# hal9000universe/deep-q-learning

Hardware: AMD Instinct MI355X
Metric: grad-updates/sec (higher is better)
Workload: dtype f32

## Files before the change

### deep-q-learning_amd/csrc/dqn_api.hip

```cpp
#include "../../include/dqn_hip.h"
#include "dqn_launch.h"
#include "dqn_per_device.h"

#include <dlfcn.h>
#include <cmath>
#include <cstdarg>
#include <cstdio>
#include <cstdlib>
#include <cstring>
#include <map>
#include <new>
#include <string>
#include <vector>

static thread_local std::string g_err;
thread_local hipEvent_t g_prof_ev0 = nullptr, g_prof_ev1 = nullptr;
static int fail(int code, const char *fmt, ...) {
    char buf[512];
    va_list ap; va_start(ap, fmt); vsnprintf(buf, sizeof(buf), fmt, ap); va_end(ap);
    g_err = buf;
    return code;
}
int dqn_set_error(int code, const char *msg) { g_err = msg; return code; }
#define HIP_TRY(expr)                                                                          \
// ... 22 lines not shown
struct Rccl {
    void *lib = nullptr;
    int (*GetUniqueId)(void *) = nullptr;
    int (*CommInitRank)(void **, int, NcclId, int) = nullptr;
    int (*AllReduce)(const void *, void *, size_t, int, int, void *, hipStream_t) = nullptr;
    int (*CommDestroy)(void *) = nullptr;
    int (*CommCount)(void *, int *) = nullptr;
    const char *(*GetErrorString)(int) = nullptr;
};

struct dqn_handle {
    dqn_config cfg;
    NetDims m;
    int L = 0;
    long long Ntree = 0;
    int Bp = 0;
    bool bf16 = false;
    void *arena = nullptr;
    size_t arena_bytes = 0, pack_bytes = 0;
    DqnState *st = nullptr;
    float *params = nullptr, *target = nullptr, *mu = nullptr, *nu = nullptr, *grad = nullptr;
    float *pack = nullptr, *pack_t = nullptr;
    float *pack_act = nullptr;
    float *states = nullptr, *observations = nullptr, *rewards = nullptr;
    int32_t *actions = nullptr; uint8_t *dones = nullptr;
    float *tree = nullptr; unsigned long long *stamp = nullptr;
    float *bs = nullptr, *bs2 = nullptr, *br = nullptr, *bw_raw = nullptr, *bisw = nullptr, *btd = nullptr,
          *btd_abs = nullptr, *bdf = nullptr;
    int32_t *ba = nullptr, *bidx = nullptr; uint8_t *bd = nullptr;
    float *q = nullptr, *nq = nullptr, *nt = nullptr;
    float *px = nullptr, *ph1 = nullptr, *ph2 = nullptr, *pdz1 = nullptr, *pdz2 = nullptr, *pdz3 = nullptr;
    float *loss_part = nullptr, *loss_dev = nullptr, *scratch = nullptr;
    int *tile_cnt = nullptr;
    float *big_slab = nullptr, *big_colsum = nullptr;
    float *pw_part = nullptr; int pw_force = 0;
    unsigned int *wmax_tmp = nullptr;
    int num_cus = 256;
    float *env_obs = nullptr, *env_next = nullptr, *env_r = nullptr; int32_t *env_a = nullptr; uint8_t *env_d = nullptr;
    float *hist_s = nullptr, *hist_r = nullptr; int32_t *hist_a = nullptr, *hist_d = nullptr;
    int n_step = 1; float gamma_n = 0.0f;
    bool no_handover = false;
    bool no_actor16 = false, f32_actor = false;
    bool big_any = false;
    int withhold = 0;
    int tile_stride = 0;
    float p_done = 0.01f;
    int env_kind = 0, env_max_steps = 500; int32_t *env_t = nullptr; float env_term_reward = 1.0f;
    bool env_time_feature = false;
    bool profiling = false;
    std::vector<hipEvent_t> events; size_t ev_used = 0;
    std::vector<const char *> ev_names;
    std::map<int, GraphSet> graphs;
    std::map<std::vector<int>, hipGraphExec_t> loop_graphs;
    void *comm = nullptr; int rank = 0, world = 1;
    std::map<int, std::pair<void *, int64_t>> bufs;
};

static Rccl g_rccl;

static size_t align_up(size_t x, size_t a) { return (x + a - 1) / a * a; }

static void L_pack(dqn_handle *h, hipStream_t s, const float *params, float *pack) {
    if (h->bf16) {
        launch_pack_bf16(s, h->m, params, pack);
        if (pack == h->pack) { launch_pack(s, h->m, params, h->pack_act); launch_pack_w2k16(s, h->m, params, h->pack_act); }
    } else launch_pack(s, h->m, params, pack);
}
static bool big_from(const dqn_handle *h, int B) { return h->big_any || (h->bf16 && B >= DQN_BIG_MIN_BF16); }
static bool use_big(dqn_handle *h, int B) { return h->big_slab != nullptr && big_supported(h->m, B, big_from(h, B)); }
static void L_fwd(dqn_handle *h, hipStream_t s, const FwdPass *p, int n, int B, const SampleArgs *smp = nullptr,
                  const BwdArgs *fuse = nullptr) {
    if (use_big(h, B) && !smp && !fuse) {
        bool plain = true;
        for (int i = 0; i < n; ++i) plain = plain && !p[i].act_out && !p[i].px && p[i].x;
        if (plain) { if (h->bf16) launch_big16_forward(s, h->m, p, n, B, h->num_cus); else launch_big_forward(s, h->m, p, n, B, h->num_cus); return; }
    }
    if (h->bf16) launch_qnet_fwd_bf16(s, h->m, p, n, B, smp, fuse, h->tile_cnt, h->st, h->tile_stride, h->withhold);
    else launch_qnet_fwd(s, h->m, p, n, B, smp, fuse, h->tile_cnt, h->st, h->tile_stride, h->withhold);
}
static void L_bwd(dqn_handle *h, hipStream_t s, const BwdArgs &g, int B) {
    if (h->bf16) launch_bwd_rows_bf16(s, h->m, g, B, h->st); else launch_bwd_rows(s, h->m, g, B, h->st);
}
static void L_dw(dqn_handle *h, hipStream_t s, int B, float *loss_out, int bump, const AdamArgs &ad, const PwArgs &pw) {
    if (h->bf16) launch_dw_bf16(s, h->m, h->px, h->ph1, h->ph2, h->pdz1, h->pdz2, h->pdz3, B, h->grad, h->loss_part, loss_out, h->st, bump, ad, pw);
    else launch_dw(s, h->m, h->px, h->ph1, h->ph2, h->pdz1, h->pdz2, h->pdz3, B, h->grad, h->loss_part, loss_out, h->st, bump, ad, pw);
}

static void arm(dqn_handle *h) {
    if (!h->profiling) return;
    while (h->events.size() < h->ev_used + 2) {
        hipEvent_t e;
        if (hipEventCreate(&e) != hipSuccess) return;
        h->events.push_back(e);
    }
    g_prof_ev0 = h->events[h->ev_used]; g_prof_ev1 = h->events[h->ev_used + 1];
}
static void mark(dqn_handle *h, hipStream_t st, const char *name) {
    (void)st;
    if (!h->profiling) return;
    h->ev_used += 2;
    h->ev_names.push_back(name);
}

extern "C" int dqn_create(const dqn_config *cfg, dqn_handle **out) {
    REQUIRE(cfg && out, "dqn_create: null argument");
    const int D = cfg->obs_dim, H1 = cfg->hidden1, H2 = cfg->hidden2, A = cfg->num_actions;
    REQUIRE(D >= 1 && D <= 256, "obs_dim %d out of range [1,256]", D);
    REQUIRE(H1 >= 16 && H1 <= 256 && H1 % 16 == 0, "hidden1 %d must be a multiple of 16 in [16,256]", H1);
    REQUIRE(H2 >= 16 && H2 <= 256 && H2 % 16 == 0, "hidden2 %d must be a multiple of 16 in [16,256]", H2);
    REQUIRE(A >= 1 && A <= 15, "num_actions %d out of range [1,15]", A);
    REQUIRE(cfg->capacity >= 1 && cfg->capacity <= (1ll << 30), "capacity out of range");
// ... 31 lines not shown
        if (L < 1) L = 1;
        h->L = L; h->Ntree = 1ll << L;
    }
    const long long N = cfg->capacity, P = h->m.P, Bp = h->Bp;
    const int K1 = h->m.KQ1 * 16;

    struct Item { void **p; size_t bytes; int id; };
    std::vector<Item> items;
    auto add = [&](void *pp, size_t bytes, int id = -1) { items.push_back({(void **)pp, bytes, id}); };
    add(&h->st, sizeof(DqnState));
    add(&h->params, P * 4, DQN_BUF_PARAMS); add(&h->target, P * 4, DQN_BUF_TARGET);
    add(&h->mu, P * 4, DQN_BUF_MU); add(&h->nu, P * 4, DQN_BUF_NU); add(&h->grad, P * 4, DQN_BUF_GRAD);
    const size_t esz = h->bf16 ? 2 : 4;
    const size_t pack_bytes = h->bf16 ? (size_t)bf16_pack_elems(h->m) * 2 : (size_t)h->m.pack_floats * 4;
    h->pack_bytes = pack_bytes;
    add(&h->pack, pack_bytes); add(&h->pack_t, pack_bytes);
    if (h->bf16) add(&h->pack_act, (size_t)h->m.pack_floats * 4 + (size_t)h->m.H1 * h->m.H2 * 2);
    add(&h->states, N * D * 4, DQN_BUF_STATES); add(&h->observations, N * D * 4, DQN_BUF_OBSERVATIONS);
    add(&h->rewards, N * 4, DQN_BUF_REWARDS); add(&h->actions, N * 4, DQN_BUF_ACTIONS);
    add(&h->dones, N, DQN_BUF_DONES);
    if (cfg->use_per) { add(&h->tree, 2 * h->Ntree * 4, DQN_BUF_TREE); add(&h->stamp, h->Ntree * 8); add(&h->pw_part, 8192 * 4); }
    add(&h->bs, Bp * D * 4); add(&h->bs2, Bp * D * 4); add(&h->br, Bp * 4); add(&h->bw_raw, Bp * 4);
    add(&h->bisw, Bp * 4, DQN_BUF_BATCH_ISW); add(&h->btd, Bp * 4, DQN_BUF_BATCH_TD); add(&h->btd_abs, Bp * 4);
    add(&h->bdf, Bp * 4); add(&h->ba, Bp * 4); add(&h->bidx, Bp * 4, DQN_BUF_BATCH_IDX); add(&h->bd, Bp);
    add(&h->q, Bp * A * 4); add(&h->nq, Bp * A * 4); add(&h->nt, Bp * A * 4);
    add(&h->px, Bp * (h->bf16 ? 32 : K1) * esz);
    add(&h->ph1, Bp * H1 * esz); add(&h->ph2, Bp * H2 * esz);
    add(&h->pdz1, Bp * H1 * esz); add(&h->pdz2, Bp * H2 * esz); add(&h->pdz3, Bp * 16 * esz);
    add(&h->loss_part, (Bp / 16) * 4); add(&h->loss_dev, 4, DQN_BUF_LOSS); add(&h->scratch, Bp * 4);
    if (big_supported(h->m, cfg->max_batch, big_from(h, cfg->max_batch))) {
        add(&h->big_slab, big_slab_floats(cfg->max_batch, h->num_cus) * 4); add(&h->big_colsum, big_colsum_floats(cfg->max_batch) * 4);
    }
    h->tile_stride = (int)(Bp / 16) + 2;
    add(&h->tile_cnt, (size_t)h->tile_stride * 2 * 4); add(&h->wmax_tmp, 4);
    add(&h->env_obs, Bp * D * 4, DQN_BUF_ENV_OBS); add(&h->env_next, Bp * D * 4); add(&h->env_r, Bp * 4);
    add(&h->env_a, Bp * 4, DQN_BUF_ENV_ACTIONS); add(&h->env_d, Bp); add(&h->env_t, Bp * 4);
    if (h->n_step > 1) {
        const size_t ns = (size_t)h->n_step;
        add(&h->hist_s, ns * Bp * D * 4); add(&h->hist_r, ns * Bp * 4); add(&h->hist_a, ns * Bp * 4); add(&h->hist_d, ns * Bp * 4);
    }
    size_t total = 0;
    for (auto &it : items) total += align_up(it.bytes, 256);
    hipError_t e = hipMalloc(&h->arena, total);
    if (e != hipSuccess) { delete h; return fail(DQN_ERR_NOMEM, "hipMalloc(%zu bytes): %s", total, hipGetErrorString(e)); }
    h->arena_bytes = total;
    e = hipMemset(h->arena, 0, total);
    if (e != hipSuccess) { (void)hipFree(h->arena); delete h; return fail(DQN_ERR_HIP, "hipMemset: %s", hipGetErrorString(e)); }
    size_t off = 0;
    for (auto &it : items) {
        *it.p = (char *)h->arena + off;
        if (it.id >= 0) h->bufs[it.id] = {*it.p, (int64_t)it.bytes};
        off += align_up(it.bytes, 256);
    }
    DqnState s0{};
    s0.b1pow = 1.0; s0.b2pow = 1.0; s0.pmax = 1.0f; s0.beta = cfg->per_beta; s0.lr = cfg->lr;
    e = hipMemcpy(h->st, &s0, sizeof(s0), hipMemcpyHostToDevice);
    if (e != hipSuccess) { (void)hipFree(h->arena); delete h; return fail(DQN_ERR_HIP, "state init: %s", hipGetErrorString(e)); }
    *out = h;
    return DQN_OK;
}

static void destroy_graphs(dqn_handle *h) {
    for (auto &kv : h->graphs) {
        if (kv.second.fused) (void)hipGraphExecDestroy(kv.second.fused);
        if (kv.second.bwd) (void)hipGraphExecDestroy(kv.second.bwd);
        if (kv.second.apply) (void)hipGraphExecDestroy(kv.second.apply);
        if (kv.second.actor) (void)hipGraphExecDestroy(kv.second.actor);
// ... 341 lines not shown
            mark(h, st, "big_fwd2");
            g.nq = h->nq; g.nt = h->nt;
            arm(h);
            launch_big16_rows_bwd(st, h->m, p + 2, 1, B, g, h->px, h->ph1, h->ph2, h->big_colsum, h->st, h->num_cus);
        } else launch_big_rows_bwd(st, h->m, p, 3, B, g, h->px, h->ph1, h->ph2, h->big_colsum, h->st, h->num_cus);
        mark(h, st, "big_rows_fwd3_bwd");
        arm(h);
        (h->bf16 ? launch_big16_dw : launch_big_dw)(st, h->m, h->px, h->ph1, h->ph2, h->pdz1, h->pdz2, h->pdz3, B, h->big_slab, h->big_colsum, h->grad,
                      h->loss_part, h->loss_dev, h->st, 1, fuse_adam ? adam_args(h) : AdamArgs{}, h->num_cus);
        mark(h, st, "big_dw");
        if (fuse_pw && h->cfg.use_per) enqueue_per_writeback(h, B, st);
        (void)defer_top;
        return;
    }
    SampleArgs sm{};
    sm.st = h->st; sm.tree = h->cfg.use_per ? h->tree : nullptr; sm.N = h->Ntree; sm.L = h->L;
    sm.states = h->states; sm.observations = h->observations; sm.rewards = h->rewards; sm.actions = h->actions;
    sm.dones = h->dones; sm.seed = h->cfg.seed;
    sm.idx = h->bidx; sm.a = h->ba; sm.r = h->br; sm.w_raw = h->bw_raw; sm.d = h->bd;
    sm.pre = presampled ? 1 : 0;
    FwdPass p[3] = { make_pass(h, DQN_NET_ONLINE, nullptr, h->q, nullptr, true),
                     make_pass(h, DQN_NET_ONLINE, nullptr, h->nq, nullptr, false),
                     make_pass(h, DQN_NET_TARGET, nullptr, h->nt, nullptr, false) };
    p[0].src = 1; p[1].src = 2; p[2].src = 2;
    BwdArgs g{};
    g.q = h->q; g.nq = h->nq; g.nt = h->nt; g.a = h->ba; g.r = h->br; g.d_u8 = h->bd;
    g.w_raw = h->cfg.use_per ? h->bw_raw : nullptr;
    g.gamma = h->n_step > 1 ? h->gamma_n : h->cfg.gamma;
    g.ph1 = h->ph1; g.ph2 = h->ph2; g.pack = h->pack;
    g.pdz1 = h->pdz1; g.pdz2 = h->pdz2; g.pdz3 = h->pdz3;
    g.td = h->btd; g.td_abs = h->btd_abs; g.isw_out = h->bisw; g.loss_part = h->loss_part;
    const int grid_tiles = h->bf16 ? 2 * ((B + 31) / 32) : (B + 15) / 16;
    const bool fuse_rows = 3 * grid_tiles <= h->num_cus && (presampled || !h->cfg.use_per) && !h->no_handover;
    if (fuse_rows) p[0].q = nullptr;
    arm(h);
    L_fwd(h, st, p, 3, B, &sm, fuse_rows ? &g : nullptr);
    mark(h, st, fuse_rows ? "sample_fwd_x3_bwd" : "sample_fwd_x3");
    if (!fuse_rows) {
        arm(h);
        L_bwd(h, st, g, B);
        mark(h, st, "td_bwd_rows");
    }
    PwArgs pw{};
    if (fuse_pw && h->cfg.use_per)
        pw = PwArgs{h->tree, h->Ntree, h->L, h->bidx, h->btd_abs, B, h->cfg.per_alpha, h->cfg.per_eps};
    arm(h);
    L_dw(h, st, B, h->loss_dev, 1, fuse_adam ? adam_args(h) : AdamArgs{}, pw);
    mark(h, st, fuse_adam ? (pw.tree ? "dw_adam_perwrite" : "dw_adam") : (pw.tree ? "dw_perwrite" : "dw"));
    if (pw.tree && !defer_top) { arm(h); launch_per_top(st, h->st, h->tree, h->L); mark(h, st, "per_top"); }
}

static void enqueue_apply(dqn_handle *h, int B, hipStream_t st) {
    (void)B;
    arm(h);
    enqueue_adam(h, st);
    mark(h, st, "adam");
}

static void enqueue_update(dqn_handle *h, int B, hipStream_t st, bool capturing, bool defer_top = false,
                           bool presampled = false) {
    (void)capturing;
    if (h->world == 1) {
        enqueue_backward(h, B, st, true, true, defer_top, presampled);
    } else {
        enqueue_backward(h, B, st, false, true, false, presampled);
        enqueue_apply(h, B, st);
    }
// ... 310 lines not shown

extern "C" int dqn_allreduce_grads(dqn_handle *h, void *stream) {
    REQUIRE(h, "null argument");
    if (!h->comm) return fail(DQN_ERR_STATE, "dqn_allreduce_grads before dqn_comm_init");
    const int e = g_rccl.AllReduce(h->grad, h->grad, (size_t)h->m.P,  7,  0, h->comm,
                                   (hipStream_t)stream);
    if (e) return fail(DQN_ERR_COMM, "ncclAllReduce: %s", g_rccl.GetErrorString ? g_rccl.GetErrorString(e) : "?");
    return DQN_OK;
}

extern "C" int dqn_comm_count_host(dqn_handle *h, int32_t *ranks) {
    REQUIRE(h && ranks, "null argument");
    *ranks = 0;
    if (!h->comm) return DQN_OK;
    if (!g_rccl.CommCount) return fail(DQN_ERR_COMM, "librccl.so lacks ncclCommCount");
    int n = 0;
    const int e = g_rccl.CommCount(h->comm, &n);
    if (e) return fail(DQN_ERR_COMM, "ncclCommCount: %s", g_rccl.GetErrorString ? g_rccl.GetErrorString(e) : "?");
    *ranks = n;
    return DQN_OK;
}

extern "C" int dqn_debug_withhold_handover(dqn_handle *h, int32_t on) {
    REQUIRE(h, "null handle");
    HIP_TRY(hipDeviceSynchronize());
    destroy_graphs(h);
    h->withhold = on ? 1 : 0;
    return DQN_OK;
}

extern "C" int dqn_clear_device_errors(dqn_handle *h) {
    REQUIRE(h, "null handle");
    HIP_TRY(hipDeviceSynchronize());
    if (h->tile_cnt) HIP_TRY(hipMemset(h->tile_cnt, 0, (size_t)h->tile_stride * 2 * 4));
    const unsigned int z = 0;
    HIP_TRY(hipMemcpy(&h->st->err_count, &z, 4, hipMemcpyHostToDevice));
    HIP_TRY(hipMemcpy(&h->st->arrive, &z, 4, hipMemcpyHostToDevice));
    HIP_TRY(hipMemcpy(&h->st->fill_cnt, &z, 4, hipMemcpyHostToDevice));
    return DQN_OK;
}

extern "C" int dqn_device_errors_host(dqn_handle *h, int64_t *count) {
    REQUIRE(h && count, "null argument");
    unsigned int c = 0;
    HIP_TRY(hipDeviceSynchronize());
    HIP_TRY(hipMemcpy(&c, &h->st->err_count, 4, hipMemcpyDeviceToHost));
    *count = (int64_t)c;
    return DQN_OK;
}
```

### deep-q-learning_amd/csrc/dqn_device.h

```cpp
#pragma once
#include <hip/hip_runtime.h>
#include <stdint.h>

#define LDS_BARRIER() asm volatile("s_waitcnt lgkmcnt(0)\n\ts_barrier" ::: "memory")

struct DqnState {
    unsigned long long ring_counter;
    long long          size;
    unsigned long long sample_ctr;
    unsigned long long epoch;
    unsigned long long env_ctr;
    double             b1pow, b2pow;
    int                adam_count;
    float              pmax;
    float              beta;
    float              lr;
    float              loss;
    float              wmax;
    float              epsilon;
    float              pad0;
    unsigned int       arrive;
    unsigned int       pad;
    unsigned long long ep_count;
    unsigned long long ep_steps;
// ... 58 lines not shown
    p = p * z; p = p + 1.0f;
    const float ln_m = (2.0f * s) * p;
    const float r = ln_m * 1.44269502f;
    return (float)e + r;
}

__device__ __forceinline__ float exp2_det(float y) {
    const float fi = floorf(y + 0.5f);
    int i = (int)fi;
    const float f = y - fi;
    const float t = f * 0.693147182f;
    float p = 1.98412701e-4f;
    p = p * t; p = p + 1.38888892e-3f;
    p = p * t; p = p + 8.33333377e-3f;
    p = p * t; p = p + 4.16666679e-2f;
    p = p * t; p = p + 0.166666672f;
    p = p * t; p = p + 0.5f;
    p = p * t; p = p + 1.0f;
    p = p * t; p = p + 1.0f;
    i = i < -126 ? -126 : (i > 127 ? 127 : i);
    return p * __uint_as_float((uint32_t)(i + 127) << 23);
}

__device__ __forceinline__ float pow_det(float x, float a) { return exp2_det(a * log2_det(x)); }

__device__ __forceinline__ unsigned int ticket_take_early(unsigned int *p, unsigned int v) {
    __attribute__((address_space(1))) unsigned int *g = (__attribute__((address_space(1))) unsigned int *)p;
    asm volatile("" : "+v"(g));
    return __hip_atomic_fetch_add(g, v, __ATOMIC_RELAXED, __HIP_MEMORY_SCOPE_AGENT);
}

#ifdef DQN_STAMPS
extern __device__ unsigned long long g_stamps[8][64][2];
#define STAMP(K, S)                                                                         \
    do { if (threadIdx.x == 0 && blockIdx.x == 0 && blockIdx.y == 0) {                       \
             g_stamps[K][S][0] = __builtin_amdgcn_s_memtime();                                \
             g_stamps[K][S][1] = __builtin_amdgcn_s_memrealtime(); } } while (0)
#else
#define STAMP(K, S) do { } while (0)

#endif
```

### deep-q-learning_amd/csrc/dqn_launch.h

```cpp
#pragma once
#include <hip/hip_runtime.h>
#include <stdint.h>
#include "dqn_device.h"

#include <hip/hip_ext.h>

int dqn_set_error(int code, const char *msg);

struct EnvArgs;
struct SampleArgs;

extern thread_local hipEvent_t g_prof_ev0, g_prof_ev1;
#define DQN_LAUNCH(kernel, grid, block, lds, stream, ...)                                                    \
    do {                                                                                                      \
        if (g_prof_ev0) {                                                                                     \
            hipExtLaunchKernelGGL(kernel, grid, block, lds, stream, g_prof_ev0, g_prof_ev1, 0, __VA_ARGS__); \
            g_prof_ev0 = nullptr; g_prof_ev1 = nullptr;                                                       \
        } else {                                                                                              \
            hipLaunchKernelGGL(kernel, grid, block, lds, stream, __VA_ARGS__);                                \
        }                                                                                                     \
    } while (0)

struct NetDims {
    int D, H1, H2, A;
// ... 1 lines not shown
    long long o_w1, o_b1, o_w2, o_b2, o_wv, o_bv, o_wa, o_ba, P;
    long long p_w1, p_w2, p_wh, p_w2t, p_wht, pack_floats;
    long long p_w2k;
};
NetDims make_dims(int D, int H1, int H2, int A);

struct FwdPass {
    const float *x;
    const float *params;
    const float *pack;
    float *q;
    float *feat;
    float *px, *ph1, *ph2;
    int src;
    int32_t *act_out;
    const DqnState *act_state;
    float act_eps; unsigned long long act_seed, act_ctr;
};

struct BwdArgs {
    const float *q, *nq, *nt;
    const float *targets;
    const int32_t *a; const float *r; const uint8_t *d_u8; const float *d_f32;
    const float *w_raw;
    const float *isw;
    float gamma;
    const float *ph1, *ph2;
    const float *pack;
    float *pdz1, *pdz2, *pdz3;
    float *td, *td_abs, *dq, *targets_out, *isw_out;
    float *loss_part;
};

struct FuseBwd { BwdArgs g; int *tile_cnt; DqnState *st; int tiles; int withhold; };

struct PwArgs {
    float *tree; long long N; int L; const int32_t *idx; const float *td_abs; int B; float alpha, eps;
};
struct AdamArgs {
    float *P, *mu, *nu, *pack; int adamw; float b1, b2, eps, wd, grad_scale;
    float *pack_act;
};

void launch_pack(hipStream_t s, const NetDims &m, const float *params, float *pack);
void launch_pack_w2k16(hipStream_t s, const NetDims &m, const float *params, float *pack_act);
void launch_qnet_fwd(hipStream_t s, const NetDims &m, const FwdPass *passes, int npass, int B, const SampleArgs *smp = nullptr,
                     const BwdArgs *fuse = nullptr, int *tile_cnt = nullptr, DqnState *st = nullptr, int tile_stride = 0, int withhold = 0);
bool actor_multi_supported(const NetDims &m, int n_envs, int T);
bool launch_actor_multi(hipStream_t s, const NetDims &m, const EnvArgs &env, int T, const float *params, const float *pack,
                        int32_t *act_out, int B, const SampleArgs *smp, bool bf16, int num_cus, bool no_wide);
void launch_td(hipStream_t s, const float *q, const float *nq, const float *nt, const int32_t *a,
               const float *r, const float *d, const float *isw, float gamma, int B, int A,
               float *targets, float *td, float *dq, float *loss, float *scratch);
void launch_loss(hipStream_t s, const float *pred, const float *targets, const float *isw, int B, int A,
                 float *loss);
void launch_bwd_rows(hipStream_t s, const NetDims &m, const BwdArgs &g, int B, DqnState *st);
void launch_dw(hipStream_t s, const NetDims &m, const float *px, const float *ph1, const float *ph2,
               const float *pdz1, const float *pdz2, const float *pdz3, int B, float *grad,
               const float *loss_part, float *loss_out, DqnState *st, int bump_ctr, const AdamArgs &adam,
               const PwArgs &pw = PwArgs{});
void launch_per_top(hipStream_t st_, DqnState *st, float *tree, int L);
void launch_adam(hipStream_t s, const NetDims &m, DqnState *st, float *params, const float *grad, float *mu,
                 float *nu, float *pack, int adamw, float b1, float b2, float eps, float wd, float grad_scale);
void launch_policy(hipStream_t s, const float *q, int n, int A, float epsilon, unsigned long long seed,
                   unsigned long long ctr, int32_t *actions, const DqnState *st_from);
void launch_u8_to_f32(hipStream_t s, const uint8_t *in, float *out, int n);

#define DQN_BIG_MIN 16384
#define DQN_BIG_MIN_BF16 8192
#define DQN_BIG_MAX_SLICES 64
bool big_supported(const NetDims &m, int B, bool any_size = false);
size_t big_slab_floats(int max_batch, int num_cus);
size_t big_colsum_floats(int max_batch);
int big_dw_slices(int B, int num_cus);
int dqn_rccl_comm_init(void **comm, const void *unique_id_128, int rank, int world);
int dqn_rccl_allreduce_sum_f32(void *comm, float *buf, size_t n, hipStream_t st);
void dqn_rccl_comm_destroy(void *comm);
int dqn_rccl_comm_count(void *comm, int *n);
void launch_big_forward(hipStream_t s, const NetDims &m, const FwdPass *passes, int npass, int B, int num_cus);
void launch_big16_forward(hipStream_t s, const NetDims &m, const FwdPass *passes, int npass, int B, int num_cus);
// ... 47 lines not shown
```

### deep-q-learning_amd/csrc/dqn_net.hip

```cpp
#include <type_traits>
#include "dqn_device.h"
#include "dqn_launch.h"
#include "dqn_per_device.h"
#include "dqn_net_common.h"


#ifdef DQN_STAMPS
__device__ unsigned long long g_stamps[8][64][2];
extern "C" int dqn_debug_stamps(unsigned long long *out_host) {
    return (int)hipMemcpyFromSymbol(out_host, HIP_SYMBOL(g_stamps), sizeof(g_stamps));
}
#endif

#define MFMA4(a, b, c) __builtin_amdgcn_mfma_f32_16x16x4f32((a), (b), (c), 0, 0, 0)

__device__ __forceinline__ int perm16(int c) { return ((c & 3) << 2) | (c >> 2); }


__device__ __forceinline__ int pfrag(int KQb, int tile, int ct, int r, int lane) {
    return (ct * KQb + tile) * 256 + r * 64 + ((lane & 15) << 2) + (lane >> 4);
}

NetDims make_dims(int D, int H1, int H2, int A) {
    NetDims m{};
// ... 57 lines not shown
struct MmaLayer {
    static constexpr int AHEAD = PF >= 16 ? 6 : PF;
    const float4 *pk[TN];
    float4 b0[PF][TN], b1[PP ? PF : 1][PP ? TN : 1];
    int KQ, CT, wave;

    template <int R, int C>
    __device__ __forceinline__ void load(float4 (&b)[R][C], int kq0) {
#pragma unroll
        for (int p = 0; p < PF; ++p) {
            int kq = kq0 + p;
            kq = kq < KQ ? kq : KQ - 1;
#pragma unroll
            for (int t = 0; t < TN; ++t) b[p][t] = pk[t][(long long)kq * 64];
        }
    }
    template <int R, int C>
    __device__ __forceinline__ void compute(const float4 (&b)[R][C], int kq0, const float *arow, f32x4 (&acc)[TN]) {
#pragma unroll
        for (int p = 0; p < PF; ++p) {
            const int kq = kq0 + p;
            if (kq < KQ) {
                const float4 a4 = *reinterpret_cast<const float4 *>(arow + 16 * kq);
#pragma unroll
                for (int t = 0; t < TN; ++t) {
                    acc[t] = MFMA4(a4.x, b[p][t].x, acc[t]);
                    acc[t] = MFMA4(a4.y, b[p][t].y, acc[t]);
                    acc[t] = MFMA4(a4.z, b[p][t].z, acc[t]);
                    acc[t] = MFMA4(a4.w, b[p][t].w, acc[t]);
                }
            }
        }
    }
    __device__ __forceinline__ void init(const float *__restrict__ pack, int KQ_, int CT_, int wave_, int lane) {
        KQ = KQ_; CT = CT_; wave = wave_;
#pragma unroll
        for (int t = 0; t < TN; ++t) {
            int ct = wave + 4 * t;
            ct = ct < CT ? ct : CT - 1;
            pk[t] = reinterpret_cast<const float4 *>(pack) + (long long)ct * KQ * 64 + lane;
        }
    }
    template <int P0, int P1>
    __device__ __forceinline__ void load_range() {
#pragma unroll
        for (int p = P0; p < P1; ++p) {
            int kq = p < KQ ? p : KQ - 1;
#pragma unroll
            for (int t = 0; t < TN; ++t) b0[p][t] = pk[t][(long long)kq * 64];
        }
    }
    __device__ __forceinline__ void start(const float *__restrict__ pack, int KQ_, int CT_, int wave_, int lane) {
        init(pack, KQ_, CT_, wave_, lane);
        load(b0, 0);
    }
    __device__ __forceinline__ void finish_heads4(const float *lds_a, int stride, int lane, f32x4 &out) {
        static_assert(TN == 1 && !PP, "heads: one tile, single chunk");
        f32x4 c0 = {0.f, 0.f, 0.f, 0.f}, c1 = c0, c2 = c0, c3 = c0;
        const float *arow = lds_a + (lane & 15) * stride + 4 * (lane >> 4);
        float4 a_cur = *reinterpret_cast<const float4 *>(arow);
#pragma unroll
        for (int p = 0; p < PF; ++p) {
            if (p < KQ) {
                const float4 a4 = a_cur;
                if (p + 1 < PF) a_cur = *reinterpret_cast<const float4 *>(arow + (p + 1 < KQ ? 16 * (p + 1) : 0));
                c0 = MFMA4(a4.x, b0[p][0].x, c0);
                c1 = MFMA4(a4.y, b0[p][0].y, c1);
                c2 = MFMA4(a4.z, b0[p][0].z, c2);
                c3 = MFMA4(a4.w, b0[p][0].w, c3);
                __builtin_amdgcn_sched_barrier(0);
            }
// ... 41 lines not shown
struct FwdPasses { FwdPass p[3]; };


template <int TN1, int TN2, bool FUSE>
__global__ void __launch_bounds__(256)
k_qnet_fwd(NetDims m, FwdPasses passes, int B, SampleArgs smp, FuseBwd fb) {
    extern __shared__ __attribute__((aligned(16))) float lds[];
    const FwdPass ps = passes.p[blockIdx.y];
    const int tile = blockIdx.x, row0 = tile * 16;
    const int tid = threadIdx.x, wave = tid >> 6, lane = tid & 63;
    const int KQb = (B + 15) / 16;
    const int K1 = m.KQ1 * 16;
    const int sx = K1 + 4, s1 = m.H1 + 4, s2 = m.H2 + 4;
    float *lx = lds, *l1 = lx + 16 * sx, *l2 = l1 + 16 * s1, *lh = l2 + 16 * s2;

    STAMP(0, 0);
    const bool sampling = smp.st != nullptr;
    int *lidx = reinterpret_cast<int *>(lh + 256 + 16);
    const float *ring = sampling ? (ps.src == 1 ? smp.states : smp.observations) : nullptr;
    auto xload = [&](int t) -> float {
        const int rl = t / K1, c = t - rl * K1;
        if (!(t < 16 * K1 && row0 + rl < B && c < m.D)) return 0.0f;
        return sampling ? ring[(long long)lidx[rl] * m.D + c] : ps.x[(long long)(row0 + rl) * m.D + c];
    };
    float xv[4];
    if (!sampling) {
#pragma unroll
        for (int u = 0; u < 4; ++u) xv[u] = xload(tid + 256 * u);
    }
    const bool presampled = sampling && smp.pre;
    int pre_leaf = 0;
    if (presampled && tid < 16) pre_leaf = smp.idx[row0 + tid < B ? row0 + tid : B - 1];
    MmaLayer<TN1, 2, true> L1; MmaLayer<TN2, 16, false> L2; MmaLayer<1, 16, false> LH;
    MmaLayer<TN2, 1, false> LA; MmaLayer<TN1, 16, false> LB;
    L1.start(ps.pack + m.p_w1, m.KQ1, m.H1 / 16, wave, lane);
    float bias1[TN1], bias2[TN2], biash = 0.0f;
#pragma unroll
    for (int t = 0; t < TN1; ++t) { int ct = wave + 4 * t; ct = ct < m.H1 / 16 ? ct : m.H1 / 16 - 1; bias1[t] = ps.params[m.o_b1 + 16 * ct + (lane & 15)]; }
#pragma unroll
    for (int t = 0; t < TN2; ++t) { int ct = wave + 4 * t; ct = ct < m.H2 / 16 ? ct : m.H2 / 16 - 1; bias2[t] = ps.params[m.o_b2 + 16 * ct + (lane & 15)]; }
    if (wave == 0) {
        const int c = lane & 15;
        if (c == 0) biash = ps.params[m.o_bv];
        else if (c <= m.A) biash = ps.params[m.o_ba + c - 1];
    }
    int row_a = 0; float row_r = 0.0f; int row_d = 0;
    if (presampled) {
        if (tid < 16) {
            lidx[tid] = pre_leaf;
            const int k = row0 + tid;
            if (blockIdx.y == 0 && k < B) {
                row_a = smp.actions[pre_leaf]; row_r = smp.rewards[pre_leaf]; row_d = smp.dones[pre_leaf];
                smp.a[k] = row_a; smp.r[k] = row_r; smp.d[k] = (uint8_t)row_d;
            }
        }
        LDS_BARRIER();
#pragma unroll
        for (int u = 0; u < 4; ++u) xv[u] = xload(tid + 256 * u);
    }
    L2.init(ps.pack + m.p_w2, m.H1 / 16, m.H2 / 16, wave, lane);
    L2.template load_range<0, 6>();
    if (wave == 0) LH.init(ps.pack + m.p_wh, m.H2 / 16, 1, 0, lane);
    if (sampling && !presampled) {
        if (smp.tree) {
            float *lsub = reinterpret_cast<float *>(lidx + 16);
            sample_tile_coop(smp, row0, B, tid, blockIdx.y == 0, lidx, lsub, lsub + 512);
        } else {
            if (tid < 16) sample_tile(smp, row0, B, tid, blockIdx.y == 0, lidx);
            LDS_BARRIER();
        }
#pragma unroll
        for (int u = 0; u < 4; ++u) xv[u] = xload(tid + 256 * u);
        if constexpr (FUSE) {
            if (blockIdx.y == 0 && tid < 16 && row0 + tid < B) {
                const int leaf = lidx[tid];
                row_a = smp.actions[leaf]; row_r = smp.rewards[leaf]; row_d = smp.dones[leaf];
            }
        }
    }

#pragma unroll
    for (int u = 0; u < 4; ++u) {
        const int t = tid + 256 * u;
        if (t < 16 * K1) {
            const int rl = t / K1, c = t - rl * K1;
            lx[rl * sx + (c & ~15) + perm16(c & 15)] = xv[u];
        }
    }
    for (int t = tid + 1024; t < 16 * K1; t += 256) {
        const int rl = t / K1, c = t - rl * K1;
        const float v = xload(t);
        lx[rl * sx + (c & ~15) + perm16(c & 15)] = v;
    }
    LDS_BARRIER();
    STAMP(0, 1);

    unsigned m1bits = 0u, m2bits = 0u;
    {
        f32x4 acc[TN1];
        L1.finish(lx, sx, lane, acc);
        STAMP(0, 11);
#pragma unroll
        for (int t = 0; t < TN1; ++t) {
            const int ct = wave + 4 * t;
            if (ct < m.H1 / 16) {
                const int c = lane & 15;
                const float bias = bias1[t];
// ... 6 lines not shown
                    l1[rl * s1 + 16 * ct + perm16(c)] = v;
                }
            }
        }
    }
    STAMP(0, 12);
    if (wave == 0) LH.template load_range<0, 16>();
    STAMP(0, 13);
    LDS_BARRIER();
    STAMP(0, 2);

    {
        f32x4 acc[TN2];
        L2.finish(l1, s1, lane, acc);
        STAMP(0, 3);
#pragma unroll
        for (int t = 0; t < TN2; ++t) {
            const int ct = wave + 4 * t;
            if (ct < m.H2 / 16) {
                const int c = lane & 15, col = 16 * ct + c;
                const float bias = bias2[t];
#pragma unroll
                for (int r = 0; r < 4; ++r) {
                    const int rl = 4 * (lane >> 4) + r;
                    float v = acc[t][r] + bias;
                    v = v > 0.0f ? v : 0.0f;
                    if constexpr (FUSE) m2bits |= (v > 0.0f ? 1u : 0u) << (4 * t + r);
                    l2[rl * s2 + 16 * ct + perm16(c)] = v;
                    if (ps.feat && row0 + rl < B) ps.feat[(long long)(row0 + rl) * m.H2 + col] = v;
                }
            }
        }
    }
    LDS_BARRIER();
    STAMP(0, 4);

    if (ps.px && wave != 0) {
        auto stash = [&](float *dst, const float *img, int stride, int CT) {
            float4 *out = reinterpret_cast<float4 *>(dst);
            for (int q = tid - 64; q < CT * 64; q += 192) {
                const int ct = q >> 6, lp = q & 63;
                const float *col = img + (lp >> 4) * stride + 16 * ct + perm16(lp & 15);
                out[(long long)(ct * KQb + tile) * 64 + lp] = float4{col[0], col[4 * stride], col[8 * stride], col[12 * stride]};
            }
        };
        stash(ps.px, lx, sx, m.KQ1);
        stash(ps.ph1, l1, s1, m.H1 / 16);
        stash(ps.ph2, l2, s2, m.H2 / 16);
    }
    if (wave == 0) {
        f32x4 acc;
        LH.finish_heads4(l2, s2, lane, acc);
        const int c = lane & 15;
#pragma unroll
        for (int r = 0; r < 4; ++r) lh[(4 * (lane >> 4) + r) * 16 + c] = acc[r] + biash;
    }
    if constexpr (FUSE) {
        if (blockIdx.y == 0) {
            LA.start(fb.g.pack + m.p_wht, 1, m.H2 / 16, wave, lane);
            LB.init(fb.g.pack + m.p_w2t, m.H2 / 16, m.H1 / 16, wave, lane);
            LB.template load_range<0, 16>();
        }
    }
    LDS_BARRIER();
    STAMP(0, 5);

    float qrow[16];
    if (tid < 16 && row0 + tid < B) {
        const float *hr = lh + tid * 16;
        float sum = 0.0f;
        if constexpr (FUSE) {
            if (m.A <= 4) {
#pragma unroll
                for (int a = 0; a < 4; ++a) if (a < m.A) sum = sum + hr[1 + a];
            } else {
#pragma unroll
                for (int a = 0; a < 15; ++a) if (a < m.A) sum = sum + hr[1 + a];
            }
        } else {
            for (int a = 0; a < m.A; ++a) sum = sum + hr[1 + a];
        }
        const float mean = __fdiv_rn(sum, (float)m.A);
        if constexpr (FUSE) {
#pragma unroll
            for (int a = 0; a < 15; ++a) qrow[a] = a < m.A ? (hr[0] + hr[1 + a]) - mean : 0.0f;
        } else {
            for (int a = 0; a < m.A; ++a) qrow[a] = (hr[0] + hr[1 + a]) - mean;
        }
        if constexpr (FUSE) {
            if (blockIdx.y != 0) {
#pragma unroll
                for (int a = 0; a < 15; ++a) asm volatile("" : "+v"(qrow[a]));
#pragma unroll
                for (int a = 0; a < 15; ++a)
                    if (a < m.A) __hip_atomic_store(&ps.q[(long long)(row0 + tid) * m.A + a], qrow[a], __ATOMIC_RELAXED, __HIP_MEMORY_SCOPE_AGENT);
            } else if (ps.q) {
#pragma unroll
                for (int a = 0; a < 15; ++a) if (a < m.A) ps.q[(long long)(row0 + tid) * m.A + a] = qrow[a];
            }
        } else if (ps.q) for (int a = 0; a < m.A; ++a) ps.q[(long long)(row0 + tid) * m.A + a] = qrow[a];
        if (ps.act_out) {
            const float eps = ps.act_state ? ps.act_state->epsilon : ps.act_eps;
            const unsigned long long ctr = ps.act_state ? ps.act_state->env_ctr : ps.act_ctr;
            const int act = policy_row(qrow, m.A, eps, ps.act_seed, ctr, row0 + tid);
            ps.act_out[row0 + tid] = act;
        }
    }
    STAMP(0, 6);
    if constexpr (FUSE) {
        if (blockIdx.y != 0) {
            if (wave == 0) {
                asm volatile("s_waitcnt vmcnt(0)" ::: "memory");
                if (tid == 0) atomicAdd(reinterpret_cast<unsigned *>(fb.tile_cnt) + tile, fb.withhold ? 0u : 1u);
            }
            return;
        }
        const BwdArgs &g = fb.g;
        const int A = m.A;
        const int s3 = 16 + 4;
        float *l3 = lx;
        float *lz2 = lh + 256 + 32 + 528, *lrow = lz2 + 16 * s2;
        const int irow = row0 + tid;
        const bool rowt = tid < 16 && irow < B;
        float wi = 1.0f, wmax = 1.0f;
        if (rowt && g.w_raw) { wi = g.w_raw[irow]; wmax = fb.st->wmax; }
        for (int t = tid; t < 16 * s3; t += 256) l3[t] = 0.0f;
        bool gave_up = false;
        if (tid == 0) {
            unsigned *cnt = reinterpret_cast<unsigned *>(fb.tile_cnt) + tile, *seen = reinterpret_cast<unsigned *>(fb.tile_cnt) + fb.tiles + tile;
            const unsigned want = *seen + 2u;
            if (!wait_word_eq(cnt, want, 2)) { flag_wait_timeout(fb.st); gave_up = true; }
            *seen = want;
        }
        LDS_BARRIER();
        STAMP(0, 7);
        if (tid < 16) {
            float rowloss = 0.0f;
            if (rowt) {
                auto td_rows = [&](auto amax_tag) {
                constexpr int AMAX = decltype(amax_tag)::value;
                float nqr[AMAX], ntr[AMAX];
#pragma unroll
                for (int k2 = 0; k2 < AMAX; ++k2) {
                    nqr[k2] = k2 < A ? __hip_atomic_load(&g.nq[(long long)irow * A + k2], __ATOMIC_RELAXED, __HIP_MEMORY_SCOPE_AGENT) : 0.0f;
                    ntr[k2] = k2 < A ? __hip_atomic_load(&g.nt[(long long)irow * A + k2], __ATOMIC_RELAXED, __HIP_MEMORY_SCOPE_AGENT) : 0.0f;
                }
                float w = 1.0f;
                if (g.w_raw) w = __fdiv_rn(wi, wmax);
                const float invB = __fdiv_rn(1.0f, (float)B);
                float best = nqr[0], nt_star = ntr[0], q_a = qrow[0];
#pragma unroll
                for (int k2 = 1; k2 < AMAX; ++k2) {
                    if (k2 < A && nqr[k2] > best) { best = nqr[k2]; nt_star = ntr[k2]; }
                    if (k2 == row_a) q_a = qrow[k2];
                }
                const float di = row_d ? 1.0f : 0.0f;
                const float t1 = g.gamma * nt_star;
                const float t2 = t1 - q_a;
                const float t3 = (1.0f - di) * t2;
                float delta = row_r + t3, dabs = fabsf(delta);
                asm volatile("" : "+v"(delta), "+v"(dabs), "+v"(w));
                if (g.w_raw && g.isw_out) g.isw_out[irow] = w;
                if (g.td) g.td[irow] = delta;
                if (g.td_abs) g.td_abs[irow] = dabs;
                float gk[AMAX], gsum = 0.0f;
#pragma unroll
                for (int k2 = 0; k2 < AMAX; ++k2) {
                    gk[k2] = 0.0f;
                    if (k2 < A) {
                        const float trk = qrow[k2] + delta * (k2 == row_a ? 1.0f : 0.0f);
                        const float e = qrow[k2] - trk;
                        rowloss = rowloss + huber(e);
                        const float c = e > 1.0f ? 1.0f : (e < -1.0f ? -1.0f : e);
                        gk[k2] = (w * c) * invB;
                        gsum = gsum + gk[k2];
                        if (g.dq) g.dq[(long long)irow * A + k2] = gk[k2];
                        if (g.targets_out) g.targets_out[(long long)irow * A + k2] = trk;
                    }
                }
                if (g.w_raw) rowloss = w * rowloss;
                const float gmean = __fdiv_rn(gsum, (float)A);
                l3[tid * s3 + perm16(0)] = gsum;
#pragma unroll
                for (int k2 = 0; k2 < AMAX; ++k2) if (k2 < A) l3[tid * s3 + perm16(1 + k2)] = gk[k2] - gmean;
                };
                if (A <= 4) td_rows(std::integral_constant<int, 4>{}); else td_rows(std::integral_constant<int, 15>{});
            }
            lrow[tid] = rowloss;
        }
        LDS_BARRIER();
        STAMP(0, 8);
        if (tid == 0) {
            float sl = 0.0f;
            for (int k = 0; k < 16; ++k) sl = sl + lrow[k];
            g.loss_part[tile] = gave_up ? __int_as_float(0x7fc00000) : sl;
        }
        {
            const int rl = tid >> 4, c = tid & 15;
            g.pdz3[pidx(KQb, row0 + rl, c)] = l3[rl * s3 + perm16(c)];
        }
        {
            f32x4 acc[TN2];
            LA.finish(l3, s3, lane, acc);
#pragma unroll
            for (int t = 0; t < TN2; ++t) {
                const int ct = wave + 4 * t;
                if (ct < m.H2 / 16) {
                    const int c = lane & 15;
#pragma unroll
                    for (int r = 0; r < 4; ++r) {
                        const int rl = 4 * (lane >> 4) + r;
                        const float v = ((m2bits >> (4 * t + r)) & 1u) ? acc[t][r] : 0.0f;
                        lz2[rl * s2 + 16 * ct + perm16(c)] = v;
                        g.pdz2[pfrag(KQb, tile, ct, r, lane)] = v;
                    }
                }
            }
        }
        LDS_BARRIER();
        STAMP(0, 9);
        {
            f32x4 acc[TN1];
            LB.finish(lz2, s2, lane, acc, true);
#pragma unroll
            for (int t = 0; t < TN1; ++t) {
                const int ct = wave + 4 * t;
                if (ct < m.H1 / 16) {
#pragma unroll
                    for (int r = 0; r < 4; ++r) g.pdz1[pfrag(KQb, tile, ct, r, lane)] = ((m1bits >> (4 * t + r)) & 1u) ? acc[t][r] : 0.0f;
                }
            }
        }
        STAMP(0, 10);
    }
}

static inline int tn_of(int H) { const int ct = H / 16; return ct <= 4 ? 1 : (ct <= 8 ? 2 : 4); }

void launch_qnet_fwd(hipStream_t s, const NetDims &m, const FwdPass *passes, int npass, int B, const SampleArgs *smp,
                     const BwdArgs *fuse, int *tile_cnt, DqnState *st, int tile_stride, int withhold) {
    FwdPasses ps{};
    for (int i = 0; i < npass; ++i) ps.p[i] = passes[i];
    const SampleArgs sa = smp ? *smp : SampleArgs{};
    const dim3 grid((B + 15) / 16, npass), block(256);
    size_t lds = sizeof(float) * (16 * (m.KQ1 * 16 + 4) + 16 * (m.H1 + 4) + 16 * (m.H2 + 4) + 256 + 32 + 528);
    const int t1 = tn_of(m.H1), t2 = tn_of(m.H2);
    if (fuse) {
        FuseBwd fb{*fuse, tile_cnt, st, tile_stride, withhold};
        lds += sizeof(float) * (16 * (m.H2 + 4) + 16);
#define FWD_CASE(A1, A2) if (t1 == A1 && t2 == A2) { DQN_LAUNCH((k_qnet_fwd<A1, A2, true>), grid, block, lds, s, m, ps, B, sa, fb); return; }
        FWD_CASE(1, 1) FWD_CASE(1, 2) FWD_CASE(1, 4) FWD_CASE(2, 1) FWD_CASE(2, 2) FWD_CASE(2, 4)
        FWD_CASE(4, 1) FWD_CASE(4, 2) FWD_CASE(4, 4)
#undef FWD_CASE
    }
    const FuseBwd fb{};
#define FWD_CASE(A1, A2) if (t1 == A1 && t2 == A2) { DQN_LAUNCH((k_qnet_fwd<A1, A2, false>), grid, block, lds, s, m, ps, B, sa, fb); return; }
    FWD_CASE(1, 1) FWD_CASE(1, 2) FWD_CASE(1, 4) FWD_CASE(2, 1) FWD_CASE(2, 2) FWD_CASE(2, 4)
    FWD_CASE(4, 1) FWD_CASE(4, 2) FWD_CASE(4, 4)
#undef FWD_CASE
}

__global__ void __launch_bounds__(256)
k_td(const float *__restrict__ q, const float *__restrict__ nq, const float *__restrict__ nt,
     const int32_t *__restrict__ a, const float *__restrict__ r, const float *__restrict__ d,
     const float *__restrict__ isw, float gamma, int B, int A, float *targets, float *td, float *dq,
     float *scratch) {
    const int i = blockIdx.x * blockDim.x + threadIdx.x;
    if (i >= B) return;
    float qr[16], nqr[16], ntr[16], tr[16];
    for (int k = 0; k < A; ++k) { qr[k] = q[(long long)i * A + k]; nqr[k] = nq[(long long)i * A + k]; ntr[k] = nt[(long long)i * A + k]; }
    const float delta = td_row(qr, nqr, ntr, a[i], r[i], d[i], gamma, A, tr);
    const float w = isw ? isw[i] : 1.0f;
    const float invB = __fdiv_rn(1.0f, (float)B);
    float row = 0.0f;
    for (int k = 0; k < A; ++k) {
        const float e = qr[k] - tr[k];
        row = row + huber(e);
        const float c = e > 1.0f ? 1.0f : (e < -1.0f ? -1.0f : e);
        if (dq) dq[(long long)i * A + k] = (w * c) * invB;
        if (targets) targets[(long long)i * A + k] = tr[k];
    }
// ... 421 lines not shown
```

Measured before the change: 17380.

## Split fused backward dz1/dz2 work across the two target-pass blocks

```diff
diff --git a/deep-q-learning_amd/csrc/dqn_api.hip b/deep-q-learning_amd/csrc/dqn_api.hip
--- a/deep-q-learning_amd/csrc/dqn_api.hip
+++ b/deep-q-learning_amd/csrc/dqn_api.hip
@@ -78,6 +78,7 @@
     float *px = nullptr, *ph1 = nullptr, *ph2 = nullptr, *pdz1 = nullptr, *pdz2 = nullptr, *pdz3 = nullptr;
     float *loss_part = nullptr, *loss_dev = nullptr, *scratch = nullptr;
     int *tile_cnt = nullptr;
+    unsigned long long *gates = nullptr;
     float *big_slab = nullptr, *big_colsum = nullptr;
     float *pw_part = nullptr; int pw_force = 0;
     unsigned int *wmax_tmp = nullptr;
@@ -122,7 +123,7 @@
         if (plain) { if (h->bf16) launch_big16_forward(s, h->m, p, n, B, h->num_cus); else launch_big_forward(s, h->m, p, n, B, h->num_cus); return; }
     }
     if (h->bf16) launch_qnet_fwd_bf16(s, h->m, p, n, B, smp, fuse, h->tile_cnt, h->st, h->tile_stride, h->withhold);
-    else launch_qnet_fwd(s, h->m, p, n, B, smp, fuse, h->tile_cnt, h->st, h->tile_stride, h->withhold);
+    else launch_qnet_fwd(s, h->m, p, n, B, smp, fuse, h->tile_cnt, h->st, h->tile_stride, h->withhold, h->gates);
 }
 static void L_bwd(dqn_handle *h, hipStream_t s, const BwdArgs &g, int B) {
     if (h->bf16) launch_bwd_rows_bf16(s, h->m, g, B, h->st); else launch_bwd_rows(s, h->m, g, B, h->st);
@@ -220,7 +221,8 @@
         add(&h->big_slab, big_slab_floats(cfg->max_batch, h->num_cus) * 4); add(&h->big_colsum, big_colsum_floats(cfg->max_batch) * 4);
     }
     h->tile_stride = (int)(Bp / 16) + 2;
-    add(&h->tile_cnt, (size_t)h->tile_stride * 2 * 4); add(&h->wmax_tmp, 4);
+    add(&h->tile_cnt, (size_t)h->tile_stride * 5 * 4); add(&h->wmax_tmp, 4);
+    add(&h->gates, (size_t)std::min(h->tile_stride, h->num_cus) * 2048);
     add(&h->env_obs, Bp * D * 4, DQN_BUF_ENV_OBS); add(&h->env_next, Bp * D * 4); add(&h->env_r, Bp * 4);
     add(&h->env_a, Bp * 4, DQN_BUF_ENV_ACTIONS); add(&h->env_d, Bp); add(&h->env_t, Bp * 4);
     if (h->n_step > 1) {
@@ -628,7 +630,7 @@
     g.td = h->btd; g.td_abs = h->btd_abs; g.isw_out = h->bisw; g.loss_part = h->loss_part;
     const int grid_tiles = h->bf16 ? 2 * ((B + 31) / 32) : (B + 15) / 16;
     const bool fuse_rows = 3 * grid_tiles <= h->num_cus && (presampled || !h->cfg.use_per) && !h->no_handover;
-    if (fuse_rows) p[0].q = nullptr;
+    if (fuse_rows && h->bf16) p[0].q = nullptr;
     arm(h);
     L_fwd(h, st, p, 3, B, &sm, fuse_rows ? &g : nullptr);
     mark(h, st, fuse_rows ? "sample_fwd_x3_bwd" : "sample_fwd_x3");
@@ -1005,7 +1007,7 @@
 extern "C" int dqn_clear_device_errors(dqn_handle *h) {
     REQUIRE(h, "null handle");
     HIP_TRY(hipDeviceSynchronize());
-    if (h->tile_cnt) HIP_TRY(hipMemset(h->tile_cnt, 0, (size_t)h->tile_stride * 2 * 4));
+    if (h->tile_cnt) HIP_TRY(hipMemset(h->tile_cnt, 0, (size_t)h->tile_stride * 5 * 4));
     const unsigned int z = 0;
     HIP_TRY(hipMemcpy(&h->st->err_count, &z, 4, hipMemcpyHostToDevice));
     HIP_TRY(hipMemcpy(&h->st->arrive, &z, 4, hipMemcpyHostToDevice));
diff --git a/deep-q-learning_amd/csrc/dqn_device.h b/deep-q-learning_amd/csrc/dqn_device.h
--- a/deep-q-learning_amd/csrc/dqn_device.h
+++ b/deep-q-learning_amd/csrc/dqn_device.h
@@ -114,11 +114,13 @@
 
 #ifdef DQN_STAMPS
 extern __device__ unsigned long long g_stamps[8][64][2];
-#define STAMP(K, S)                                                                         \
-    do { if (threadIdx.x == 0 && blockIdx.x == 0 && blockIdx.y == 0) {                       \
+#define STAMP_Y(K, S, Y)                                                                    \
+    do { if (threadIdx.x == 0 && blockIdx.x == 0 && blockIdx.y == (Y)) {                     \
              g_stamps[K][S][0] = __builtin_amdgcn_s_memtime();                                \
              g_stamps[K][S][1] = __builtin_amdgcn_s_memrealtime(); } } while (0)
+#define STAMP(K, S) STAMP_Y(K, S, 0)
 #else
+#define STAMP_Y(K, S, Y) do { } while (0)
 #define STAMP(K, S) do { } while (0)
 
 #endif
diff --git a/deep-q-learning_amd/csrc/dqn_launch.h b/deep-q-learning_amd/csrc/dqn_launch.h
--- a/deep-q-learning_amd/csrc/dqn_launch.h
+++ b/deep-q-learning_amd/csrc/dqn_launch.h
@@ -57,7 +57,7 @@
     float *loss_part;
 };
 
-struct FuseBwd { BwdArgs g; int *tile_cnt; DqnState *st; int tiles; int withhold; };
+struct FuseBwd { BwdArgs g; int *tile_cnt; DqnState *st; int tiles; int withhold; unsigned long long *gates; };
 
 struct PwArgs {
     float *tree; long long N; int L; const int32_t *idx; const float *td_abs; int B; float alpha, eps;
@@ -70,7 +70,8 @@
 void launch_pack(hipStream_t s, const NetDims &m, const float *params, float *pack);
 void launch_pack_w2k16(hipStream_t s, const NetDims &m, const float *params, float *pack_act);
 void launch_qnet_fwd(hipStream_t s, const NetDims &m, const FwdPass *passes, int npass, int B, const SampleArgs *smp = nullptr,
-                     const BwdArgs *fuse = nullptr, int *tile_cnt = nullptr, DqnState *st = nullptr, int tile_stride = 0, int withhold = 0);
+                     const BwdArgs *fuse = nullptr, int *tile_cnt = nullptr, DqnState *st = nullptr, int tile_stride = 0, int withhold = 0,
+                     unsigned long long *gates = nullptr);
 bool actor_multi_supported(const NetDims &m, int n_envs, int T);
 bool launch_actor_multi(hipStream_t s, const NetDims &m, const EnvArgs &env, int T, const float *params, const float *pack,
                         int32_t *act_out, int B, const SampleArgs *smp, bool bf16, int num_cus, bool no_wide);
diff --git a/deep-q-learning_amd/csrc/dqn_net.hip b/deep-q-learning_amd/csrc/dqn_net.hip
--- a/deep-q-learning_amd/csrc/dqn_net.hip
+++ b/deep-q-learning_amd/csrc/dqn_net.hip
@@ -113,11 +113,11 @@
             }
         }
     }
-    __device__ __forceinline__ void init(const float *__restrict__ pack, int KQ_, int CT_, int wave_, int lane) {
+    __device__ __forceinline__ void init(const float *__restrict__ pack, int KQ_, int CT_, int wave_, int lane, int ct0 = 0) {
         KQ = KQ_; CT = CT_; wave = wave_;
 #pragma unroll
         for (int t = 0; t < TN; ++t) {
-            int ct = wave + 4 * t;
+            int ct = ct0 + wave + 4 * t;
             ct = ct < CT ? ct : CT - 1;
             pk[t] = reinterpret_cast<const float4 *>(pack) + (long long)ct * KQ * 64 + lane;
         }
@@ -225,7 +225,8 @@
     int pre_leaf = 0;
     if (presampled && tid < 16) pre_leaf = smp.idx[row0 + tid < B ? row0 + tid : B - 1];
     MmaLayer<TN1, 2, true> L1; MmaLayer<TN2, 16, false> L2; MmaLayer<1, 16, false> LH;
-    MmaLayer<TN2, 1, false> LA; MmaLayer<TN1, 16, false> LB;
+    constexpr int TNH = TN1 > 1 ? TN1 / 2 : 1;
+    MmaLayer<TN2, 1, false> LA; MmaLayer<TNH, 16, false> LB;
     L1.start(ps.pack + m.p_w1, m.KQ1, m.H1 / 16, wave, lane);
     float bias1[TN1], bias2[TN2], biash = 0.0f;
 #pragma unroll
@@ -242,10 +243,10 @@
         if (tid < 16) {
             lidx[tid] = pre_leaf;
             const int k = row0 + tid;
-            if (blockIdx.y == 0 && k < B) {
+            if ((FUSE || blockIdx.y == 0) && k < B) {
                 row_a = smp.actions[pre_leaf]; row_r = smp.rewards[pre_leaf]; row_d = smp.dones[pre_leaf];
-                smp.a[k] = row_a; smp.r[k] = row_r; smp.d[k] = (uint8_t)row_d;
-            }
+            }
+            if (blockIdx.y == 0 && k < B) { smp.a[k] = row_a; smp.r[k] = row_r; smp.d[k] = (uint8_t)row_d; }
         }
         LDS_BARRIER();
 #pragma unroll
@@ -265,7 +266,7 @@
 #pragma unroll
         for (int u = 0; u < 4; ++u) xv[u] = xload(tid + 256 * u);
         if constexpr (FUSE) {
-            if (blockIdx.y == 0 && tid < 16 && row0 + tid < B) {
+            if (tid < 16 && row0 + tid < B) {
                 const int leaf = lidx[tid];
                 row_a = smp.actions[leaf]; row_r = smp.rewards[leaf]; row_d = smp.dones[leaf];
             }
@@ -338,6 +339,11 @@
             }
         }
     }
+    if constexpr (FUSE) {
+        if (blockIdx.y == 0)
+            __hip_atomic_store(fb.gates + tile * 256 + tid, (unsigned long long)m1bits | ((unsigned long long)m2bits << 32),
+                               __ATOMIC_RELAXED, __HIP_MEMORY_SCOPE_AGENT);
+    }
     LDS_BARRIER();
     STAMP(0, 4);
 
@@ -361,13 +367,6 @@
 #pragma unroll
         for (int r = 0; r < 4; ++r) lh[(4 * (lane >> 4) + r) * 16 + c] = acc[r] + biash;
     }
-    if constexpr (FUSE) {
-        if (blockIdx.y == 0) {
-            LA.start(fb.g.pack + m.p_wht, 1, m.H2 / 16, wave, lane);
-            LB.init(fb.g.pack + m.p_w2t, m.H2 / 16, m.H1 / 16, wave, lane);
-            LB.template load_range<0, 16>();
-        }
-    }
     LDS_BARRIER();
     STAMP(0, 5);
 
@@ -394,15 +393,12 @@
             for (int a = 0; a < m.A; ++a) qrow[a] = (hr[0] + hr[1 + a]) - mean;
         }
         if constexpr (FUSE) {
-            if (blockIdx.y != 0) {
+            {
 #pragma unroll
                 for (int a = 0; a < 15; ++a) asm volatile("" : "+v"(qrow[a]));
 #pragma unroll
                 for (int a = 0; a < 15; ++a)
                     if (a < m.A) __hip_atomic_store(&ps.q[(long long)(row0 + tid) * m.A + a], qrow[a], __ATOMIC_RELAXED, __HIP_MEMORY_SCOPE_AGENT);
-            } else if (ps.q) {
-#pragma unroll
-                for (int a = 0; a < 15; ++a) if (a < m.A) ps.q[(long long)(row0 + tid) * m.A + a] = qrow[a];
             }
         } else if (ps.q) for (int a = 0; a < m.A; ++a) ps.q[(long long)(row0 + tid) * m.A + a] = qrow[a];
         if (ps.act_out) {
@@ -414,18 +410,28 @@
     }
     STAMP(0, 6);
     if constexpr (FUSE) {
-        if (blockIdx.y != 0) {
-            if (wave == 0) {
-                asm volatile("s_waitcnt vmcnt(0)" ::: "memory");
-                if (tid == 0) atomicAdd(reinterpret_cast<unsigned *>(fb.tile_cnt) + tile, fb.withhold ? 0u : 1u);
-            }
-            return;
+        asm volatile("s_waitcnt vmcnt(0)" ::: "memory");
+        LDS_BARRIER();
+        unsigned *cnt_all = reinterpret_cast<unsigned *>(fb.tile_cnt);
+        if (tid == 0) {
+            if (blockIdx.y != 0) atomicAdd(cnt_all + tile, fb.withhold ? 0u : 1u);
+            atomicAdd(cnt_all + 2 * fb.tiles + tile, 1u);
         }
         const BwdArgs &g = fb.g;
         const int A = m.A;
         const int s3 = 16 + 4;
+        const int half = blockIdx.y - 1;
+        const bool do_dz1 = TN1 > 1 || half == 0, store_dz2 = TN2 > 1 || half == 0;
+        if (blockIdx.y != 0 && !do_dz1 && !store_dz2) return;
         float *l3 = lx;
         float *lz2 = lh + 256 + 32 + 528, *lrow = lz2 + 16 * s2;
+        if (blockIdx.y != 0) {
+            LA.start(g.pack + m.p_wht, 1, m.H2 / 16, wave, lane);
+            if (do_dz1) {
+                LB.init(g.pack + m.p_w2t, m.H2 / 16, m.H1 / 16, wave, lane, 4 * TNH * half);
+                LB.template load_range<0, 16>();
+            }
+        }
         const int irow = row0 + tid;
         const bool rowt = tid < 16 && irow < B;
         float wi = 1.0f, wmax = 1.0f;
@@ -433,16 +439,23 @@
         for (int t = tid; t < 16 * s3; t += 256) l3[t] = 0.0f;
         bool gave_up = false;
         if (tid == 0) {
-            unsigned *cnt = reinterpret_cast<unsigned *>(fb.tile_cnt) + tile, *seen = reinterpret_cast<unsigned *>(fb.tile_cnt) + fb.tiles + tile;
-            const unsigned want = *seen + 2u;
+            unsigned *cnt = blockIdx.y == 0 ? cnt_all + tile : cnt_all + 2 * fb.tiles + tile;
+            unsigned *seen = cnt_all + (blockIdx.y == 0 ? 1 : 3 + half) * fb.tiles + tile;
+            const unsigned want = *seen + (blockIdx.y == 0 ? 2u : 3u);
             if (!wait_word_eq(cnt, want, 2)) { flag_wait_timeout(fb.st); gave_up = true; }
             *seen = want;
         }
         LDS_BARRIER();
-        STAMP(0, 7);
+        if (blockIdx.y == 0) STAMP(0, 7); else STAMP_Y(0, 16, 1);
         if (tid < 16) {
             float rowloss = 0.0f;
             if (rowt) {
+                if (blockIdx.y != 0) {
+#pragma unroll
+                    for (int k2 = 0; k2 < 15; ++k2)
+                        qrow[k2] = k2 < A ? __hip_atomic_load(&g.q[(long long)irow * A + k2], __ATOMIC_RELAXED, __HIP_MEMORY_SCOPE_AGENT) : 0.0f;
+                }
+                const bool outs = blockIdx.y == 0;
                 auto td_rows = [&](auto amax_tag) {
                 constexpr int AMAX = decltype(amax_tag)::value;
                 float nqr[AMAX], ntr[AMAX];
@@ -466,9 +479,11 @@
                 const float t3 = (1.0f - di) * t2;
                 float delta = row_r + t3, dabs = fabsf(delta);
                 asm volatile("" : "+v"(delta), "+v"(dabs), "+v"(w));
-                if (g.w_raw && g.isw_out) g.isw_out[irow] = w;
-                if (g.td) g.td[irow] = delta;
-                if (g.td_abs) g.td_abs[irow] = dabs;
+                if (outs) {
+                    if (g.w_raw && g.isw_out) g.isw_out[irow] = w;
+                    if (g.td) g.td[irow] = delta;
+                    if (g.td_abs) g.td_abs[irow] = dabs;
+                }
                 float gk[AMAX], gsum = 0.0f;
 #pragma unroll
                 for (int k2 = 0; k2 < AMAX; ++k2) {
@@ -480,8 +495,8 @@
                         const float c = e > 1.0f ? 1.0f : (e < -1.0f ? -1.0f : e);
                         gk[k2] = (w * c) * invB;
                         gsum = gsum + gk[k2];
-                        if (g.dq) g.dq[(long long)irow * A + k2] = gk[k2];
-                        if (g.targets_out) g.targets_out[(long long)irow * A + k2] = trk;
+                        if (outs && g.dq) g.dq[(long long)irow * A + k2] = gk[k2];
+                        if (outs && g.targets_out) g.targets_out[(long long)irow * A + k2] = trk;
                     }
                 }
                 if (g.w_raw) rowloss = w * rowloss;
@@ -495,16 +510,22 @@
             lrow[tid] = rowloss;
         }
         LDS_BARRIER();
-        STAMP(0, 8);
-        if (tid == 0) {
-            float sl = 0.0f;
-            for (int k = 0; k < 16; ++k) sl = sl + lrow[k];
-            g.loss_part[tile] = gave_up ? __int_as_float(0x7fc00000) : sl;
-        }
-        {
-            const int rl = tid >> 4, c = tid & 15;
-            g.pdz3[pidx(KQb, row0 + rl, c)] = l3[rl * s3 + perm16(c)];
-        }
+        if (blockIdx.y == 0) {
+            STAMP(0, 8);
+            if (tid == 0) {
+                float sl = 0.0f;
+                for (int k = 0; k < 16; ++k) sl = sl + lrow[k];
+                g.loss_part[tile] = gave_up ? __int_as_float(0x7fc00000) : sl;
+            }
+            {
+                const int rl = tid >> 4, c = tid & 15;
+                g.pdz3[pidx(KQb, row0 + rl, c)] = l3[rl * s3 + perm16(c)];
+            }
+            return;
+        }
+        STAMP_Y(0, 17, 1);
+        const unsigned long long gm = __hip_atomic_load(fb.gates + tile * 256 + tid, __ATOMIC_RELAXED, __HIP_MEMORY_SCOPE_AGENT);
+        const unsigned g1 = (unsigned)gm, g2 = (unsigned)(gm >> 32);
         {
             f32x4 acc[TN2];
             LA.finish(l3, s3, lane, acc);
@@ -513,38 +534,39 @@
                 const int ct = wave + 4 * t;
                 if (ct < m.H2 / 16) {
                     const int c = lane & 15;
+                    const bool mine = t / (TN2 > 1 ? TN2 / 2 : TN2) == half;
 #pragma unroll
                     for (int r = 0; r < 4; ++r) {
                         const int rl = 4 * (lane >> 4) + r;
-                        const float v = ((m2bits >> (4 * t + r)) & 1u) ? acc[t][r] : 0.0f;
+                        const float v = ((g2 >> (4 * t + r)) & 1u) ? acc[t][r] : 0.0f;
                         lz2[rl * s2 + 16 * ct + perm16(c)] = v;
-                        g.pdz2[pfrag(KQb, tile, ct, r, lane)] = v;
+                        if (mine) g.pdz2[pfrag(KQb, tile, ct, r, lane)] = v;
                     }
                 }
             }
         }
         LDS_BARRIER();
-        STAMP(0, 9);
-        {
-            f32x4 acc[TN1];
+        STAMP_Y(0, 18, 1);
+        if (do_dz1) {
+            f32x4 acc[TNH];
             LB.finish(lz2, s2, lane, acc, true);
 #pragma unroll
-            for (int t = 0; t < TN1; ++t) {
-                const int ct = wave + 4 * t;
-                if (ct < m.H1 / 16) {
-#pragma unroll
-                    for (int r = 0; r < 4; ++r) g.pdz1[pfrag(KQb, tile, ct, r, lane)] = ((m1bits >> (4 * t + r)) & 1u) ? acc[t][r] : 0.0f;
-                }
-            }
-        }
-        STAMP(0, 10);
+            for (int tl = 0; tl < TNH; ++tl) {
+                const int t = TNH * half + tl, ct = wave + 4 * t;
+                if (t < TN1 && ct < m.H1 / 16) {
+#pragma unroll
+                    for (int r = 0; r < 4; ++r) g.pdz1[pfrag(KQb, tile, ct, r, lane)] = ((g1 >> (4 * t + r)) & 1u) ? acc[tl][r] : 0.0f;
+                }
+            }
+        }
+        STAMP_Y(0, 19, 1);
     }
 }
 
 static inline int tn_of(int H) { const int ct = H / 16; return ct <= 4 ? 1 : (ct <= 8 ? 2 : 4); }
 
 void launch_qnet_fwd(hipStream_t s, const NetDims &m, const FwdPass *passes, int npass, int B, const SampleArgs *smp,
-                     const BwdArgs *fuse, int *tile_cnt, DqnState *st, int tile_stride, int withhold) {
+                     const BwdArgs *fuse, int *tile_cnt, DqnState *st, int tile_stride, int withhold, unsigned long long *gates) {
     FwdPasses ps{};
     for (int i = 0; i < npass; ++i) ps.p[i] = passes[i];
     const SampleArgs sa = smp ? *smp : SampleArgs{};
@@ -552,7 +574,7 @@
     size_t lds = sizeof(float) * (16 * (m.KQ1 * 16 + 4) + 16 * (m.H1 + 4) + 16 * (m.H2 + 4) + 256 + 32 + 528);
     const int t1 = tn_of(m.H1), t2 = tn_of(m.H2);
     if (fuse) {
-        FuseBwd fb{*fuse, tile_cnt, st, tile_stride, withhold};
+        FuseBwd fb{*fuse, tile_cnt, st, tile_stride, withhold, gates};
         lds += sizeof(float) * (16 * (m.H2 + 4) + 16);
 #define FWD_CASE(A1, A2) if (t1 == A1 && t2 == A2) { DQN_LAUNCH((k_qnet_fwd<A1, A2, true>), grid, block, lds, s, m, ps, B, sa, fb); return; }
         FWD_CASE(1, 1) FWD_CASE(1, 2) FWD_CASE(1, 4) FWD_CASE(2, 1) FWD_CASE(2, 2) FWD_CASE(2, 4)
```

After: 17860, median of 6. 1.03x the previous value.
